# eBay/Sequence-Semantic-Embedding

Measured on AMD Instinct MI355X. Metric: encoded seqs/sec (+ query x target cosine-scores/sec, top-1 vs ref), higher is better.
Workload: dtype f32; 1 GPU; configs[1]: classification stand-in, dual-encoder LSTM H=S=256 E=50 T=32 V=32000; encode 16384 source seqs/GPU/step + cosine top-10 vs 571-target index; batch_per_gpu=16384, seq_len=32, targets=571, parallelism=dp1, weights=random-init (reference initialisers, seed 0)

## Files before the change

sequence-semantic-embedding_amd/csrc/score_topk.hip:

```cpp
#include <cstdlib>

#include "sse_kernels.h"
#include "score_exact.h"

#define SC_THREADS 512
#define SC_KC 16
#ifndef SC_PRIO_K
#define SC_PRIO_K 1
#define SC_PRIO_E 0
#endif

#ifdef SSE_SCORE_CLOCK
#include <cstdio>
__device__ long long g_score_clk[8 * 8];
#define SC_CLK_DECL long long ck_[8] = {0, 0, 0, 0, 0, 0, 0, 0}, ck_t = clock64();
#define SC_CLK(i)                   \
  {                                 \
    const long long n_ = clock64(); \
    ck_[i] += n_ - ck_t;            \
    ck_t = n_;                      \
  }
#else
#define SC_CLK_DECL
#define SC_CLK(i)
// ... 798 lines not shown
    const int64_t blk = i >> 6;
    const int kb = (int)(blk % KB);
    const int64_t tile = blk / KB;
    const int kg = kb * 2 + (l >> 5), r = l & 31;
    f32x4 lo4 = {0, 0, 0, 0}, hi4 = {0, 0, 0, 0};
    if (kg < KG) {
      lo4 = in[((size_t)tile * KG + kg) * 64 + r];
      hi4 = in[((size_t)tile * KG + kg) * 64 + 32 + r];
    }
    const float v[8] = {lo4[0], lo4[1], lo4[2], lo4[3], hi4[0], hi4[1], hi4[2], hi4[3]};
    sse_u32x4 h, lw;
    sse_split8(v, h, lw);
    out[(size_t)blk * 128 + l] = h;
    out[(size_t)blk * 128 + 64 + l] = lw;
  }
}

hipError_t launch_frag32_to_split_bf16(const float *idxp, int64_t NT, int KG, void *out, hipStream_t stream) {
  const int KB = (KG + 1) / 2;
  const int64_t total8 = NT * KB * 64;
  if (total8 == 0) return hipSuccess;
  const int64_t blocks = (total8 + 255) / 256;
  hipLaunchKernelGGL(frag32_to_split_bf16_kernel, dim3((int)(blocks < 16384 ? blocks : 16384)), dim3(256), 0, stream,
                     reinterpret_cast<const f32x4 *>(idxp), KG, KB, total8, reinterpret_cast<sse_u32x4 *>(out));
  return hipGetLastError();
}

__device__ __forceinline__ int si_key(float f) {
  const int i = __float_as_int(f);
  return i >= 0 ? i : (i ^ 0x7FFFFFFF);
}
__device__ __forceinline__ float si_val(int k) { return __int_as_float(k >= 0 ? k : (k ^ 0x7FFFFFFF)); }
template <int CTRL, int ROWMASK>
__device__ __forceinline__ float dpp_f(float x) {
  return __int_as_float(__builtin_amdgcn_update_dpp(__float_as_int(x), __float_as_int(x), CTRL, ROWMASK, 0xF, false));
}
__device__ __forceinline__ float wave_max_f(float x) {
  x = fmaxf(x, dpp_f<0x128, 0xF>(x));
  x = fmaxf(x, dpp_f<0x124, 0xF>(x));
  x = fmaxf(x, dpp_f<0x122, 0xF>(x));
  x = fmaxf(x, dpp_f<0x121, 0xF>(x));
  x = fmaxf(x, dpp_f<0x142, 0xA>(x));
  x = fmaxf(x, dpp_f<0x143, 0xC>(x));
  return __int_as_float(__builtin_amdgcn_readlane(__float_as_int(x), 63));
}
template <int JMAX>
#ifdef SSE_SCORE_CLOCK
#define SI_CLK_PARAMS , long long (&ck_)[8], long long &ck_t
#define SI_CLK_ARGS , ck_, ck_t
#else
#define SI_CLK_PARAMS
#define SI_CLK_ARGS
#endif
__device__ __forceinline__ void si_select4(const SmallIndexArgs &a, const float *sc, int NP, int NT, int qt, int q0, int lane SI_CLK_PARAMS) {
  constexpr int QW = 4;
  const int J = (NT * 32 + 63) / 64;
  float v[QW][JMAX];
#pragma unroll
  for (int j = 0; j < JMAX; ++j) {
    const int row = lane + 64 * j;
#pragma unroll
    for (int c = 0; c < QW; ++c) v[c][j] = (j < J && row < NT * 32) ? sc[(q0 + c) * NP + row] : NEG_INF;
  }
  int lok[QW], hik[QW];
  float lm[QW];
  bool done[QW];
#pragma unroll
  for (int c = 0; c < QW; ++c) {
    float m = NEG_INF;
#pragma unroll
    for (int j = 0; j < JMAX; ++j) m = fmaxf(m, v[c][j]);
    lm[c] = m;
    lok[c] = si_key(-wave_max_f(-m));
    hik[c] = si_key(wave_max_f(m)) + 1;
    done[c] = false;
  }
  SC_CLK(5)
  for (;;) {
    bool all_done = true;
#pragma unroll
    for (int c = 0; c < QW; ++c) {
      const unsigned width = (unsigned)hik[c] - (unsigned)lok[c];
      const int mid = lok[c] + (int)(width >> 1);
      const int cnt = __popcll(__ballot(lm[c] >= si_val(mid)));
      const bool open = !done[c] && width > 1u;
      const bool ge = cnt >= SC_KC;
      lok[c] = (open && ge) ? mid : lok[c];
      hik[c] = (open && !ge) ? mid : hik[c];
      done[c] = !open || (ge && cnt <= 24);
      all_done = all_done && done[c];
    }
    if (all_done) break;
  }
  SC_CLK(6)
#pragma unroll
  for (int c = 0; c < QW; ++c) {
    const int query = qt * 32 + q0 + c;
    if (query < a.Q) {
      const float T = si_val(lok[c]);
      float cs = NEG_INF;
      int cr = -1, base = 0;
#pragma unroll
      for (int j = 0; j < JMAX; ++j) {
        const bool take = (j < J) & (v[c][j] >= T) & (v[c][j] > NEG_INF);
        const unsigned long long mask = __ballot(take);
        const int n = __popcll(mask);
        const int slot = base + (int)__builtin_amdgcn_mbcnt_hi((unsigned)(mask >> 32), __builtin_amdgcn_mbcnt_lo((unsigned)mask, 0u));
        const int dst = (take && slot < 63) ? slot : 63;
        const int gs = __builtin_amdgcn_ds_permute(dst * 4, __float_as_int(v[c][j]));
        const int gr = __builtin_amdgcn_ds_permute(dst * 4, lane + 64 * j);
        const bool recv = (lane >= base) & (lane < base + n) & (lane < 63);
        cs = recv ? __int_as_float(gs) : cs;
        cr = recv ? gr : cr;
        base += n;
      }
      const int nw = base < 63 ? base : 63;
      int rank = 0;
      for (int l = 0; l < nw; ++l) {
        const float os = __int_as_float(__builtin_amdgcn_readlane(__float_as_int(cs), l));
        const int orow = __builtin_amdgcn_readlane(cr, l);
        rank += ((os > cs) | ((os == cs) & (orow < cr))) ? 1 : 0;
      }
      const bool mine = lane < nw;
      if (mine && rank < SC_KC) {
        a.part_scores[(size_t)query * SC_KC + rank] = cs;
        a.part_ids[(size_t)query * SC_KC + rank] = cr;
      }
      if (lane >= nw && lane < SC_KC) {
        a.part_scores[(size_t)query * SC_KC + lane] = NEG_INF;
        a.part_ids[(size_t)query * SC_KC + lane] = -1;
      }
      const unsigned long long m16 = __ballot(mine && rank == SC_KC - 1);
      const float last = m16 ? __int_as_float(__builtin_amdgcn_readlane(__float_as_int(cs), __ffsll((long long)m16) - 1)) : NEG_INF;
      if (lane == 0) a.part_bnd[query] = (base > 63) ? __builtin_inff() : last;
    }
  }
}

template <int KGC>
__global__ __launch_bounds__(256) void score_small_index_kernel(SmallIndexArgs a) {
  extern __shared__ __attribute__((aligned(16))) float si_sc[];
  const int tid = threadIdx.x, lane = tid & 63, w = __builtin_amdgcn_readfirstlane(tid >> 6);
  const int NT = a.NT, NP = NT * 32 + 1;
  const int qt = blockIdx.x;
  float *sc = si_sc;
  SC_CLK_DECL
  f32x4 b[KGC];
  {
    const int row = qt * 32 + (lane & 31), kb = (lane >> 5) * 4;
    const float *src = a.q_rows + (size_t)(row < a.Q ? row : 0) * a.S + kb;
    const bool vec = (a.S & 3) == 0 && (reinterpret_cast<uintptr_t>(a.q_rows) & 15) == 0 && KGC * 8 <= a.S;
#pragma unroll
    for (int kg = 0; kg < KGC; ++kg) {
      f32x4 v = {0, 0, 0, 0};
      if (vec) {
        v = *reinterpret_cast<const f32x4 *>(src + kg * 8);
      } else {
#pragma unroll
        for (int e = 0; e < 4; ++e)
          if (kg * 8 + kb + e < a.S) v[e] = src[kg * 8 + e];
      }
      if (row >= a.Q) v = f32x4{0, 0, 0, 0};
      b[kg] = v;
    }
  }
  SC_CLK(0)
  for (int t = w; t < NT; t += 4) {
    const f32x4 *ap = reinterpret_cast<const f32x4 *>(a.idxp) + (size_t)t * KGC * 64 + lane;
    f32x16 acc = {0, 0, 0, 0, 0, 0, 0, 0, 0, 0, 0, 0, 0, 0, 0, 0};
    f32x4 ar[4];
#pragma unroll
    for (int d = 0; d < 4; ++d) ar[d] = ap[(d < KGC ? d : 0) * 64];
#pragma unroll
    for (int kg = 0; kg < KGC; ++kg) {
      __builtin_amdgcn_sched_barrier(0);
#pragma unroll
      for (int e = 0; e < 4; ++e) acc = __builtin_amdgcn_mfma_f32_32x32x2f32(ar[kg & 3][e], b[kg][e], acc, 0, 0, 0);
      __builtin_amdgcn_sched_barrier(0);
      ar[kg & 3] = ap[(kg + 4 < KGC ? kg + 4 : kg) * 64];
    }
    const int rb = t * 32 + 4 * (lane >> 5);
    float *col = sc + (lane & 31) * NP;
#pragma unroll
    for (int r = 0; r < 16; ++r) {
      const int row = rb + (r & 3) + 8 * (r >> 2);
      col[row] = (row < a.N) ? acc[r] : NEG_INF;
    }
  }
  SC_CLK(1)
  __syncthreads();
  SC_CLK(2)
  if (NT * 32 <= 640) {
    si_select4<10>(a, sc, NP, NT, qt, w * 8, lane SI_CLK_ARGS);
    SC_CLK(3)
    si_select4<10>(a, sc, NP, NT, qt, w * 8 + 4, lane SI_CLK_ARGS);
    SC_CLK(4)
#ifdef SSE_SCORE_CLOCK
    if (blockIdx.x == gridDim.x / 2 && lane == 0)
      for (int i = 0; i < 8; ++i) g_score_clk[w * 8 + i] = ck_[i];
#endif
  } else {
    si_select4<16>(a, sc, NP, NT, qt, w * 8, lane SI_CLK_ARGS);
    si_select4<16>(a, sc, NP, NT, qt, w * 8 + 4, lane SI_CLK_ARGS);
  }
}
template <int KB>
__global__ __launch_bounds__(256) void score_small_index_x3_kernel(SmallIndexArgs a) {
  extern __shared__ __attribute__((aligned(16))) float si_sc[];
  const int tid = threadIdx.x, lane = tid & 63, w = __builtin_amdgcn_readfirstlane(tid >> 6);
  const int NT = a.NT, NP = NT * 32 + 1;
  const int qt = blockIdx.x;
  float *sc = si_sc;
  SC_CLK_DECL
  sse_u32x4 bh[KB], bl[KB];
  {
    const int row = qt * 32 + (lane & 31), kb0 = (lane >> 5) * 8;
    const float *src = a.q_rows + (size_t)(row < a.Q ? row : 0) * a.S + kb0;
    const bool vec = (a.S & 3) == 0 && (reinterpret_cast<uintptr_t>(a.q_rows) & 15) == 0 && KB * 16 <= a.S;
#pragma unroll
    for (int kb = 0; kb < KB; ++kb) {
      float v[8] = {0, 0, 0, 0, 0, 0, 0, 0};
      if (vec) {
        const f32x4 v0 = *reinterpret_cast<const f32x4 *>(src + kb * 16), v1 = *reinterpret_cast<const f32x4 *>(src + kb * 16 + 4);
#pragma unroll
        for (int e = 0; e < 4; ++e) {
          v[e] = v0[e];
          v[4 + e] = v1[e];
        }
      } else {
#pragma unroll
        for (int e = 0; e < 8; ++e)
          if (kb * 16 + kb0 + e < a.S) v[e] = src[kb * 16 + e];
      }
      if (row >= a.Q) {
#pragma unroll
        for (int e = 0; e < 8; ++e) v[e] = 0.0f;
      }
      sse_split8(v, bh[kb], bl[kb]);
    }
  }
  SC_CLK(0)
  {
    constexpr int D = KB < 4 ? KB : 4;
    static_assert(KB % D == 0, "the ring index must be static");
    const sse_u32x4 *img = reinterpret_cast<const sse_u32x4 *>(a.idx_x3) + lane;
    const sse_u32x4 *ap = img + (size_t)(w < NT ? w : 0) * KB * 128;
    sse_u32x4 ah[D], al[D];
#pragma unroll
    for (int d = 0; d < D; ++d) {
      ah[d] = ap[d * 128];
      al[d] = ap[d * 128 + 64];
    }
    for (int t = w; t < NT; t += 4) {
      const sse_u32x4 *apn = img + (size_t)(t + 4 < NT ? t + 4 : t) * KB * 128;
      f32x16 acc = {0, 0, 0, 0, 0, 0, 0, 0, 0, 0, 0, 0, 0, 0, 0, 0};
#pragma unroll
      for (int kb = 0; kb < KB; ++kb) {
        __builtin_amdgcn_sched_barrier(0);
        const bf16x8_t xh = __builtin_bit_cast(bf16x8_t, ah[kb % D]), xl = __builtin_bit_cast(bf16x8_t, al[kb % D]);
        const bf16x8_t yh = __builtin_bit_cast(bf16x8_t, bh[kb]), yl = __builtin_bit_cast(bf16x8_t, bl[kb]);
        acc = __builtin_amdgcn_mfma_f32_32x32x16_bf16(xh, yh, acc, 0, 0, 0);
        acc = __builtin_amdgcn_mfma_f32_32x32x16_bf16(xh, yl, acc, 0, 0, 0);
        acc = __builtin_amdgcn_mfma_f32_32x32x16_bf16(xl, yh, acc, 0, 0, 0);
        __builtin_amdgcn_sched_barrier(0);
        const sse_u32x4 *nx = (kb + D < KB) ? ap + (kb + D) * 128 : apn + (kb + D - KB) * 128;
        ah[kb % D] = nx[0];
        al[kb % D] = nx[64];
      }
      const int rb = t * 32 + 4 * (lane >> 5);
      float *col = sc + (lane & 31) * NP;
#pragma unroll
      for (int r = 0; r < 16; ++r) {
        const int row = rb + (r & 3) + 8 * (r >> 2);
        col[row] = (row < a.N) ? acc[r] : NEG_INF;
      }
      ap = apn;
    }
  }
  SC_CLK(1)
  __syncthreads();
  SC_CLK(2)
  if (NT * 32 <= 640) {
    si_select4<10>(a, sc, NP, NT, qt, w * 8, lane SI_CLK_ARGS);
    SC_CLK(3)
    si_select4<10>(a, sc, NP, NT, qt, w * 8 + 4, lane SI_CLK_ARGS);
    SC_CLK(4)
#ifdef SSE_SCORE_CLOCK
    if (blockIdx.x == gridDim.x / 2 && lane == 0)
      for (int i = 0; i < 8; ++i) g_score_clk[w * 8 + i] = ck_[i];
#endif
  } else {
    si_select4<16>(a, sc, NP, NT, qt, w * 8, lane SI_CLK_ARGS);
    si_select4<16>(a, sc, NP, NT, qt, w * 8 + 4, lane SI_CLK_ARGS);
  }
}
bool score_small_index_applies(int Q, int KG, int64_t NT) {
  return Q >= 1024 && (KG == 32 || KG == 8 || KG == 7) && NT * 32 <= 1024 && (size_t)32 * (NT * 32 + 1) * sizeof(float) <= (size_t)144 * 1024;
}
hipError_t launch_score_small_index(const SmallIndexArgs &a, hipStream_t stream) {
  if (!score_small_index_applies(a.Q, a.KG, a.NT)) return hipErrorInvalidValue;
  const size_t lds = (size_t)32 * (a.NT * 32 + 1) * sizeof(float);
  const dim3 grid((a.Q + 31) / 32), block(256);
  auto go = [&](auto kernel) -> hipError_t {
    hipError_t e = hipFuncSetAttribute(reinterpret_cast<const void *>(kernel), hipFuncAttributeMaxDynamicSharedMemorySize, (int)lds);
    if (e != hipSuccess) return e;
    hipLaunchKernelGGL(kernel, grid, block, lds, stream, a);
    return hipGetLastError();
  };
  if (a.idx_x3 && a.KG != 32) return go(score_small_index_x3_kernel<4>);
  if (a.KG == 8) return go(score_small_index_kernel<8>);
  if (a.KG == 7) return go(score_small_index_kernel<7>);
  const hipError_t e32 = a.idx_x3 ? go(score_small_index_x3_kernel<16>) : go(score_small_index_kernel<32>);
  if (e32 != hipSuccess) return e32;
#ifdef SSE_SCORE_CLOCK
  if (a.Q >= 8192) {
    static int n = 0;
    if (n++ % 8 == 3) {
      long long v[64];
      (void)hipStreamSynchronize(stream);
      (void)hipMemcpyFromSymbol(v, HIP_SYMBOL(g_score_clk), sizeof v);
      for (int w = 0; w < 4; w += 3)
        fprintf(stderr, "[small index clock Q=%d NT=%d] wave %d cycles: query fragments %lld | scores (MFMA + LDS stores) %lld | barrier %lld | selection: loads + bounds %lld | bisection %lld | winners + rank + stores %lld (both batches)\n",
                a.Q, a.NT, w, v[w * 8 + 0], v[w * 8 + 1], v[w * 8 + 2], v[w * 8 + 5], v[w * 8 + 6], v[w * 8 + 3] + v[w * 8 + 4]);
    }
  }
#endif
  return hipGetLastError();
}

hipError_t launch_score_topk(const ScoreArgs &a_in, hipStream_t stream) {
  ScoreArgs a = a_in;
#ifdef SSE_SCORE_MEASURE
  {
    static const int dbg = getenv("SSE_SCORE_DBG") ? atoi(getenv("SSE_SCORE_DBG")) : 0;
    a.dbg = dbg;
  }
#endif
  if (a.KC != SC_KC) return hipErrorInvalidValue;
  if (a.q_rows && ((a.NQ != 1 && !a.COLLECT) || a.S < 1)) return hipErrorInvalidValue;
  if (a.NSPLIT > 8 && (a.NSPLIT & 7)) return hipErrorInvalidValue;
  if (a.NSPLIT < 8 && (8 % a.NSPLIT)) return hipErrorInvalidValue;
  if (a.COLLECT) {
    if (!a.lane_max && (!a.col_thr || !a.col_slot || !a.col_cnt || !a.col_buf)) return hipErrorInvalidValue;
    if (a.BF) return a.NQ == 4 ? launch_score_variant<4, true, true>(a, stream) : hipErrorInvalidValue;
    if (a.NQ == 1) return launch_score_variant<1, false, true>(a, stream);
    if (a.NQ == 2) return launch_score_variant<2, false, true>(a, stream);
    if (a.NQ == 4) return launch_score_variant<4, false, true>(a, stream);
    return hipErrorInvalidValue;
  }
  if (!a.part_bnd) return hipErrorInvalidValue;
  if (a.BF) {
    if (a.NQ == 1) return launch_score_variant<1, true, false>(a, stream);
    if (a.NQ == 2) return launch_score_variant<2, true, false>(a, stream);
    if (a.NQ == 4) return launch_score_variant<4, true, false>(a, stream);
    return hipErrorInvalidValue;
  }
  if (a.NQ == 1) return launch_score_variant<1, false, false>(a, stream);
  if (a.NQ == 2) return launch_score_variant<2, false, false>(a, stream);
  if (a.NQ == 4) return launch_score_variant<4, false, false>(a, stream);
  return hipErrorInvalidValue;
}


template <int NB>
__device__ __forceinline__ int packed_value_of_lane(int lane) {
  int v = 0;
#pragma unroll
  for (int cnt = NB, bit = 5; cnt > 1; cnt >>= 1, --bit) v = v * 2 + ((lane >> bit) & 1);
  return v;
}
template <int NB>
__device__ __forceinline__ int packed_lane_of_value(int v) {
  int lane = 0;
#pragma unroll
  for (int cnt = NB, bit = 5; cnt > 1; cnt >>= 1, --bit) lane |= ((v / (cnt / 2)) & 1) << bit;
  return lane;
}
template <int NB>
__device__ __forceinline__ double wave_exact_dot_packed(const float *qrow, const float *idxp, const double *idx64, const int64_t (&n)[NB],
                                                        int S, int KG, int lane, const float *idx_rm = nullptr) {
  static_assert(NB == 2 || NB == 4 || NB == 8, "power of two");
  double acc[NB];
#pragma unroll
  for (int b = 0; b < NB; ++b) acc[b] = 0.0;
  if (idx64) {
    for (int d = lane; d < S; d += 64) {
      double rv[NB];
#pragma unroll
      for (int b = 0; b < NB; ++b) rv[b] = idx64[(size_t)n[b] * S + d];
#pragma unroll
      for (int b = 0; b < NB; ++b) acc[b] += (double)qrow[d] * rv[b];
    }
  } else {
    for (int j = lane; j < KG * 2; j += 64) {
      const int kg = j >> 1, half = j & 1;
      f32x4 v[NB];
#pragma unroll
      for (int b = 0; b < NB; ++b)
        v[b] = idx_rm ? *reinterpret_cast<const f32x4 *>(idx_rm + (size_t)n[b] * S + j * 4)
                      : *reinterpret_cast<const f32x4 *>(idxp + (size_t)(n[b] >> 5) * KG * 256 + kg * 256 + (half * 32 + (int)(n[b] & 31)) * 4);
      const int d0 = kg * 8 + half * 4;
#pragma unroll
      for (int e = 0; e < 4; ++e)
        if (d0 + e < S) {
#pragma unroll
          for (int b = 0; b < NB; ++b) acc[b] += (double)qrow[d0 + e] * (double)v[b][e];
        }
    }
  }
  int m = 32;
#pragma unroll
  for (int cnt = NB; cnt > 1; cnt >>= 1, m >>= 1) {
    const bool up = (lane & m) != 0;
#pragma unroll
    for (int i = 0; i < cnt / 2; ++i) {
      const double send = up ? acc[i] : acc[i + cnt / 2];
      const double keep = up ? acc[i + cnt / 2] : acc[i];
      acc[i] = keep + __shfl_xor(send, m);
    }
  }
#pragma unroll
  for (; m > 0; m >>= 1) acc[0] += __shfl_xor(acc[0], m);
  return acc[0];
}

#define RS_THREADS 256
#define RS_MAXWIN 256
#define RS_MAXNC 4096
__global__ __launch_bounds__(RS_THREADS) void rescore_kernel(RescoreArgs a) {
  __shared__ int s_cnt;
  __shared__ int s_wid[RS_MAXWIN];
  __shared__ double s_ex[RS_MAXWIN];
  __shared__ float s_m[RS_THREADS / 64];
  __shared__ double s_qn[RS_THREADS / 64];
  extern __shared__ __attribute__((aligned(16))) unsigned long long s_key[];
  const int q = blockIdx.x, tid = threadIdx.x, lane = tid & 63, w = tid >> 6;
  if (a.uncert_clear && q == 0 && tid == 0) *a.uncert_clear = 0;
  if (a.q_count && q >= *a.q_count) return;
  const int qo = a.qmap ? a.qmap[q] : q;
  const float *ps = a.part_scores + (size_t)q * a.NC;
  const int32_t *pi = a.part_ids + (size_t)q * a.NC;
  const float *qrow = a.q + (size_t)q * a.S;
  const int KG = (a.S + 7) / 8;

  constexpr int PER = RS_MAXNC / RS_THREADS;
  float rs[PER];
  int ri[PER];
#pragma unroll
  for (int j = 0; j < PER; ++j) {
    const int c = tid + j * RS_THREADS;
    ri[j] = (c < a.NC) ? pi[c] : -1;
    rs[j] = (c < a.NC) ? ps[c] : NEG_INF;
  }
  float mmax = NEG_INF;
  for (int c = tid; c < a.NC / SC_KC; c += RS_THREADS) mmax = fmaxf(mmax, a.part_bnd[(size_t)q * (a.NC / SC_KC) + c]);

  {
    double v = 0.0;
    for (int d = tid; d < a.S; d += RS_THREADS) v += (double)qrow[d] * qrow[d];
#pragma unroll
    for (int o = 32; o > 0; o >>= 1) v += __shfl_xor(v, o);
    if (lane == 0) s_qn[w] = v;
  }
#pragma unroll
  for (int o = 32; o > 0; o >>= 1) mmax = fmaxf(mmax, __shfl_xor(mmax, o));
  if (lane == 0) s_m[w] = mmax;
  if (tid == 0) s_cnt = 0;

#pragma unroll
  for (int j = 0; j < PER; ++j) {
    const int c = tid + j * RS_THREADS;
    if (c < a.NC) {
      unsigned u = __float_as_uint(rs[j]);
      u = (u & 0x80000000u) ? ~u : (u | 0x80000000u);
      s_key[c] = (ri[j] < 0) ? 0ull : (((unsigned long long)u << 32) | (unsigned long long)(0xFFFFFFFFu - (unsigned)ri[j]));
    }
// ... 82 lines not shown
#pragma unroll
    for (int c = 0; c < 4; ++c) n[c] = s_wid[min(i0 + c, nwin - 1)];
    const double tot = wave_exact_dot_packed<4>(qrow, a.idx32, a.idx64, n, a.S, KG, lane, a.idx_rm);
    const int c = packed_value_of_lane<4>(lane);
    if ((lane & 15) == 0 && i0 + c < nwin) s_ex[i0 + c] = tot;
  }
  __syncthreads();

  double theta = -__builtin_inf();
  for (int i = tid; i < nwin; i += RS_THREADS) {
    const double s = s_ex[i];
    const int64_t id = s_wid[i];
    int rank = 0;
    for (int j = 0; j < nwin; ++j) rank += before(s_ex[j], (int64_t)s_wid[j], s, id);
    if (rank < a.k) {
      a.out_scores[(size_t)qo * a.k + rank] = s;
      a.out_ids[(size_t)qo * a.k + rank] = a.id_base + id;
      if (a.host_flag) {
        a.host_scores[(size_t)qo * a.k + rank] = s;
        a.host_ids[(size_t)qo * a.k + rank] = a.id_base + id;
      }
    }
    if (rank == a.k - 1) theta = s;
  }
  if (a.host_flag) __threadfence_system();
  {
    double t = theta;
#pragma unroll
    for (int o = 32; o > 0; o >>= 1) t = fmax(t, __shfl_xor(t, o));
    __syncthreads();
    if (lane == 0) s_ex[w] = t;
    __syncthreads();
    if (tid == 0) {
      t = fmax(fmax(s_ex[0], s_ex[1]), fmax(s_ex[2], s_ex[3]));
      const bool ok = (nwin_all <= RS_MAXWIN) && (nwin >= a.k) && ((double)mmax + (double)eps_q < t);
      a.cert[qo] = ok ? 1 : 0;
      if (!ok && a.uncert) atomicAdd(a.uncert, 1);
      if (a.col_thr) a.col_thr[qo] = ok ? __builtin_inff() : __double2float_rd(t - (double)(a.eps32 * qnorm));
      if (a.col_slot) {
        a.col_slot[qo] = ok ? -1 : qo;
        a.col_cnt[qo] = 0;
      }
      if (a.host_flag) {
        a.host_cert[qo] = ok ? 1 : 0;
        if (qo == 0 && a.host_err) *a.host_err = a.err_in ? *a.err_in : 0;
        __hip_atomic_store(a.host_flag + qo, a.seq, __ATOMIC_RELEASE, __HIP_MEMORY_SCOPE_SYSTEM);
      }
    }
  }
}

#ifndef RS_NB
#define RS_NB 4
#endif
__device__ __forceinline__ double readlane_f64(double v, int l) {
  const long long b = __double_as_longlong(v);
  const int lo = __builtin_amdgcn_readlane((int)b, l), hi = __builtin_amdgcn_readlane((int)(b >> 32), l);
  return __longlong_as_double(((long long)hi << 32) | (unsigned int)lo);
}
__global__ __launch_bounds__(256) void rescore_small_kernel(RescoreArgs a) {
  const int lane = threadIdx.x & 63;
  const int q = blockIdx.x * 4 + (threadIdx.x >> 6);
  if (a.uncert_clear && blockIdx.x == 0 && threadIdx.x == 0) *a.uncert_clear = 0;
  if (q >= a.Q) return;
  if (a.q_count && q >= *a.q_count) return;
  const int qo = a.qmap ? a.qmap[q] : q;
  const float *qrow = a.q + (size_t)q * a.S;
  const int KG = (a.S + 7) / 8;
#ifdef SSE_SCORE_CLOCK
  long long rk_[6] = {0, 0, 0, 0, 0, 0}, rk_t = clock64();
#define RS_CLK(i) { const long long n_ = clock64(); rk_[i] += n_ - rk_t; rk_t = n_; }
#else
#define RS_CLK(i)
#endif
  const bool have = lane < a.NC;
  const int id = have ? a.part_ids[(size_t)q * a.NC + lane] : -1;
  const float sc = have ? a.part_scores[(size_t)q * a.NC + lane] : NEG_INF;
  const float bnd = (lane < a.NC / SC_KC) ? a.part_bnd[(size_t)q * (a.NC / SC_KC) + lane] : NEG_INF;
  double qn = 0.0;
  for (int d = lane; d < a.S; d += 64) qn += (double)qrow[d] * qrow[d];
#pragma unroll
  for (int o = 32; o > 0; o >>= 1) qn += __shfl_xor(qn, o);
  const float qnorm = (float)sqrt(qn);
  const float eps_q = a.eps * qnorm;
  RS_CLK(0)

  unsigned u = __float_as_uint(sc);
  u = (u & 0x80000000u) ? ~u : (u | 0x80000000u);
  const unsigned long long key = (id < 0) ? 0ull : (((unsigned long long)u << 32) | (unsigned long long)(0xFFFFFFFFu - (unsigned)id));
  const int key_lo = (int)(unsigned)key, key_hi = (int)(unsigned)(key >> 32);
  int rank = 0;
  for (int j = 0; j < a.NC; ++j) {
    const unsigned long long kj = ((unsigned long long)(unsigned)__builtin_amdgcn_readlane(key_hi, j) << 32) |
                                  (unsigned long long)(unsigned)__builtin_amdgcn_readlane(key_lo, j);
    rank += (kj > key) ? 1 : 0;
  }
  const unsigned long long kmask = __ballot(key != 0ull && rank == a.k - 1);
  const float kth = kmask ? __int_as_float(__builtin_amdgcn_readlane(__float_as_int(sc), __ffsll((long long)kmask) - 1)) : NEG_INF;
  const bool in_win = (id >= 0) && (sc >= kth - 2.0f * eps_q);
  float mmax = NEG_INF;
  for (int j = 0; j < a.NC / SC_KC; ++j) mmax = fmaxf(mmax, __int_as_float(__builtin_amdgcn_readlane(__float_as_int(bnd), j)));
  const unsigned long long wmask = __ballot(in_win);
  const int nwin = __popcll(wmask);
  const int mi = __popcll(wmask & ((1ull << lane) - 1ull));
  const int idm = __builtin_amdgcn_ds_permute((in_win ? mi : 63) * 4, id);
  RS_CLK(1)
  double exm = -__builtin_inf();
  for (int m0 = 0; m0 < nwin; m0 += RS_NB) {
    int64_t n[RS_NB];
#pragma unroll
    for (int c = 0; c < RS_NB; ++c) n[c] = __builtin_amdgcn_readlane(idm, (m0 + c < nwin) ? m0 + c : 0);
    const double tot = wave_exact_dot_packed<RS_NB>(qrow, a.idx32, a.idx64, n, a.S, KG, lane, a.idx_rm);
    const int want = lane - m0;
    const double got = __shfl(tot, packed_lane_of_value<RS_NB>(want & (RS_NB - 1)));
    if (want >= 0 && want < RS_NB && lane < nwin) exm = got;
  }
  RS_CLK(2)
  int r2 = 0;
  for (int j = 0; j < nwin; ++j)
    r2 += before(readlane_f64(exm, j), (int64_t)__builtin_amdgcn_readlane(idm, j), exm, (int64_t)idm) ? 1 : 0;
  const bool member = lane < nwin;
  if (member && r2 < a.k) {
    a.out_scores[(size_t)qo * a.k + r2] = exm;
    a.out_ids[(size_t)qo * a.k + r2] = a.id_base + idm;
    if (a.host_flag) {
      a.host_scores[(size_t)qo * a.k + r2] = exm;
      a.host_ids[(size_t)qo * a.k + r2] = a.id_base + idm;
    }
  }
  const unsigned long long tmask = __ballot(member && r2 == a.k - 1);
  const double theta = tmask ? readlane_f64(exm, __ffsll((long long)tmask) - 1) : -__builtin_inf();
  if (a.host_flag) __threadfence_system();
  RS_CLK(3)
#ifdef SSE_SCORE_CLOCK
  if (q == a.Q / 2 && lane == 0) {
    rk_[4] = nwin;
    for (int i = 0; i < 6; ++i) g_score_clk[i] = rk_[i];
  }
#endif
  if (lane == 0) {
    const bool ok = (nwin >= a.k) && ((double)mmax + (double)eps_q < theta);
    a.cert[qo] = ok ? 1 : 0;
    if (!ok && a.uncert) atomicAdd(a.uncert, 1);
    if (a.col_thr) a.col_thr[qo] = ok ? __builtin_inff() : __double2float_rd(theta - (double)(a.eps32 * qnorm));
    if (a.col_slot) {
      a.col_slot[qo] = ok ? -1 : qo;
      a.col_cnt[qo] = 0;
    }
    if (a.host_flag) {
      a.host_cert[qo] = ok ? 1 : 0;
      if (qo == 0 && a.host_err) *a.host_err = a.err_in ? *a.err_in : 0;
      __hip_atomic_store(a.host_flag + qo, a.seq, __ATOMIC_RELEASE, __HIP_MEMORY_SCOPE_SYSTEM);
    }
  }
}

hipError_t launch_rescore(const RescoreArgs &a, hipStream_t stream) {
  if (a.NC > RS_MAXNC) return hipErrorInvalidValue;
  if (a.NC <= 64) {
    hipLaunchKernelGGL(rescore_small_kernel, dim3((a.Q + 3) / 4), dim3(256), 0, stream, a);
// ... 366 lines not shown
```

sequence-semantic-embedding_amd/csrc/sse_api.hip:

```cpp
#include <cmath>
#include <cstdarg>
#include <cstdio>
#include <cstdlib>
#include <algorithm>
#include <chrono>
#include <cstring>
#include <dlfcn.h>
#include <link.h>
#include <mutex>
#include <string>
#include <vector>

#include "../../include/sse_hip.h"
#include "sse_kernels.h"
#include "train.h"

namespace {

thread_local std::string g_create_error;

struct Variable {
  std::string name;
  int rows = 0, cols = 0;
  int64_t count = 0;
// ... 1534 lines not shown
  a.N = h->idx_N;
  a.Q = Q;
  a.KG = bf ? KG16 : KG;
  a.NT = (int)NT;
  a.QT = QT;
  a.NSPLIT = nsplit;
  a.KC = 16;
  a.NQ = NQ;
  if (first) {
    if (small_idx) {
      SmallIndexArgs si{q, h->idxp, a.part_scores, a.part_ids, a.part_bnd, h->idx_N, Q, S, KG, (int)NT};
      if (small_x3) si.idx_x3 = h->idx_x3.p;
      HIPCHECK(h, launch_score_small_index(si, st));
    } else {
      HIPCHECK(h, launch_score_topk(a, st));
    }
  }
  RescoreArgs r;
  r.q = q;
  r.idx32 = h->idxp;
  r.idx64 = h->idx64;
  r.idx_rm = h->idx_rm_valid ? (const float *)h->idx_rm.p : nullptr;
  r.part_scores = a.part_scores;
  r.part_ids = a.part_ids;
  r.part_bnd = a.part_bnd;
  r.out_scores = out_s;
  r.out_ids = out_i;
  r.cert = (int32_t *)h->s_cert.p;
  r.id_base = h->idx_base;
  r.N = h->idx_N;
  r.Q = Q;
  r.S = S;
  r.NC = NC;
  r.k = k;
  const float eps32 = (float)(2.0 * (S + 2) * 5.97e-8 * h->idx_norm_max);
  r.eps = eps32;
  r.eps32 = eps32;
  r.col_thr = (float *)h->s_cthr.p;
  if (first) h->uncert_word ^= 1;
  int32_t *const uncert = (int32_t *)(counters + 4) + h->uncert_word;
  const int follow_grid = 2 * (h->cu_count > 0 ? h->cu_count : 256);
  r.uncert = uncert;
  r.uncert_clear = (int32_t *)(counters + 4) + (h->uncert_word ^ 1);
  const bool own_slots = Q <= POOL;
  if (own_slots) {
    r.col_slot = (int32_t *)h->s_cslot.p;
    r.col_cnt = (int32_t *)h->s_ccnt.p;
  }
  if (bf) r.eps += (float)(1.02 * (1.0 / 256.0 + 1.0 / 262144.0) * h->idx_norm_max);
  if (small_x3)
    r.eps = (float)(((1.0 + 1.0 / 64.0) / 32768.0 + 2.0 * (3 * S + 2) * 5.97e-8 * (1.0 + 1.0 / 32.0)) * h->idx_norm_max);
  if (first) {
    RescoreArgs rf = r;
    if (mirror) {
      rf.host_scores = mirror->scores;
      rf.host_ids = mirror->ids;
      rf.host_cert = mirror->cert;
      rf.host_err = mirror->err;
      rf.host_flag = mirror->flag;
      rf.err_in = h->err_flag;
      rf.seq = mirror->seq;
    }
    HIPCHECK(h, launch_rescore(rf, st));
  }
  if (!rest) return 0;
  const float *qp32 = (const float *)h->s_qp.p;
  if (bf && Q > 32) {
    if (reserve(h, h->s_qp32, (size_t)QB * NQ * KG * 256 * sizeof(float))) return 1;
    if (reserve(h, h->s_qmap, (size_t)(Q + 1) * sizeof(int32_t))) return 1;
    if (reserve(h, h->s_qc, (size_t)QT * 32 * S * sizeof(float))) return 1;
    HIPCHECK(h, launch_count_uncert(r.cert, Q, counters, st));
    int32_t *qmap = (int32_t *)h->s_qmap.p, *qcount = qmap + Q;
    HIPCHECK(h, launch_compact_uncert(q, r.cert, Q, S, qmap, qcount, (float *)h->s_qc.p, st));
    if (!rows_direct) HIPCHECK(h, launch_pack_rows((const float *)h->s_qc.p, Q, S, (float *)h->s_qp32.p, st));
    ScoreArgs a2 = a;
    a2.BF = 0;
    a2.idxp = h->idxp;
    a2.qp = (const float *)h->s_qp32.p;
    if (rows_direct) a2.q_rows = (const float *)h->s_qc.p;
    a2.KG = KG;
    a2.q_count = qcount;
    a2.NSPLIT = nsplit2;
    HIPCHECK(h, launch_score_topk(a2, st));
    RescoreArgs r2 = r;
    r2.q = (const float *)h->s_qc.p;
    r2.NC = nsplit2 * 16;
    r2.eps = eps32;
    r2.qmap = qmap;
    r2.q_count = qcount;
    r2.uncert = r2.uncert_clear = nullptr;
    HIPCHECK(h, launch_rescore(r2, st));
    qp32 = (const float *)h->s_qp32.p;
  }
  if (!own_slots) {
    HIPCHECK(h, hipMemsetAsync(h->s_ccnt.p, 0, (size_t)(POOL + 1) * sizeof(int32_t), st));
    HIPCHECK(h, launch_assign_slots(r.cert, Q, POOL, (int32_t *)h->s_cslot.p, (int32_t *)h->s_ccnt.p + POOL, st));
  }
  ScoreArgs c = a;
  c.BF = 0;
  c.idxp = h->idxp;
  c.qp = qp32;
  c.q_rows = q;
  c.S = S;
  c.KG = KG;
  c.COLLECT = 1;
  c.col_thr = (const float *)h->s_cthr.p;
// ... 2000 lines not shown
```

sequence-semantic-embedding_amd/csrc/sse_kernels.h:

```cpp
#pragma once
#include <hip/hip_runtime.h>
#include <stdint.h>

typedef float f32x4 __attribute__((ext_vector_type(4)));
typedef float f32x16 __attribute__((ext_vector_type(16)));

__host__ __device__ static inline int frag32_off(int r_in_tile, int k_in_group) {
  return ((((k_in_group >> 2) << 5) + r_in_tile) << 2) + (k_in_group & 3);
}

__device__ static inline int mfma_row(int reg, int lane) { return (reg & 3) + 8 * (reg >> 2) + 4 * (lane >> 5); }

static inline int round_up(int x, int m) { return (x + m - 1) / m * m; }

typedef unsigned int sse_u32x4 __attribute__((ext_vector_type(4)));
__host__ __device__ static inline unsigned short sse_bf16_rne(float f) {
  unsigned u;
  __builtin_memcpy(&u, &f, 4);
  u += 0x7FFFu + ((u >> 16) & 1u);
  return (unsigned short)(u >> 16);
}
__host__ __device__ static inline float sse_bf16_f32(unsigned short h) {
  const unsigned u = (unsigned)h << 16;
  float f;
// ... 205 lines not shown
  int32_t BF = 0;
  int32_t COLLECT = 0;
  const float *col_thr = nullptr;
  const int32_t *col_slot = nullptr;
  int32_t *col_cnt = nullptr;
  int32_t *col_buf = nullptr;
  int32_t col_cap = 0;
  float *lane_max = nullptr;
  int32_t dbg = 0;
  const float *q_rows = nullptr;
  int32_t S = 0;
  const int32_t *uncert = nullptr;
};
hipError_t launch_score_topk(const ScoreArgs &a, hipStream_t stream);
hipError_t launch_lane_max_threshold(const float *q, const float *lane_max, int Q, int S, int NV, float eps, float *col_thr,
                                     int32_t *col_slot, hipStream_t st);
#define SSE_MAX_INDEX_DIM 1024
int score_pick_nq(int Q, int S, int with_bf16);
size_t score_lds_bytes(int NQ, int KG, int BF, int COLLECT);
hipError_t launch_pack_rows_bf16(const float *rows, int64_t R, int C, void *out, hipStream_t stream);
hipError_t launch_count_uncert(const int32_t *cert, int Q, unsigned long long *count, hipStream_t st);
hipError_t launch_compact_uncert(const float *q, const int32_t *cert, int Q, int S, int32_t *qmap, int32_t *count, float *qc,
                                 hipStream_t st);
hipError_t launch_frag32_to_bf16(const float *idxp, int64_t NT, int KG, void *out, hipStream_t stream);
hipError_t launch_frag32_to_split_bf16(const float *idxp, int64_t NT, int KG, void *out, hipStream_t stream);

#define SSE_COLLECT_CAP 4096
#define SSE_MAX_SELECT_K 1024

struct RescoreArgs {
  const float *q;
  const float *idx32;
  const double *idx64;
  const float *part_scores;
  const int32_t *part_ids;
  const float *part_bnd;
  double *out_scores;
  int64_t *out_ids;
  int32_t *cert;
  int64_t id_base, N;
  int32_t Q, S, NC, k;
  float eps;
  const int32_t *qmap = nullptr, *q_count = nullptr;
  float *col_thr = nullptr;
  float eps32 = 0.0f;
  int32_t *col_slot = nullptr, *col_cnt = nullptr;
  double *host_scores = nullptr;
  int64_t *host_ids = nullptr;
  int32_t *host_cert = nullptr, *host_flag = nullptr, *host_err = nullptr;
  const int32_t *err_in = nullptr;
  int32_t seq = 0;
  const float *idx_rm = nullptr;
  int32_t *uncert = nullptr, *uncert_clear = nullptr;
};
hipError_t launch_rescore(const RescoreArgs &a, hipStream_t stream);

struct SmallIndexArgs {
  const float *q_rows;
  const float *idxp;
  float *part_scores;
  int32_t *part_ids;
  float *part_bnd;
  int64_t N;
  int32_t Q, S, KG, NT;
  const void *idx_x3 = nullptr;
};
bool score_small_index_applies(int Q, int KG, int64_t NT);
hipError_t launch_score_small_index(const SmallIndexArgs &a, hipStream_t stream);

struct RankArgs {
  const float *q;
  const int32_t *pair_q;
  const int64_t *pair_id;
  const double *pair_score_in;
  const float *idxp;
  const double *idx64;
  int64_t *out_before;
  double *out_score;
  double *thr64;
  float *lo, *hi;
  unsigned long long *sure;
  int32_t *band_cnt, *band_buf;
  int32_t band_cap;
  const int32_t *bad;
  unsigned long long *counters;
  int64_t id_base, N;
  int32_t S, KG, NT, P, NSPLIT, NQ;
  float eps32;
};
hipError_t launch_rank_validate(const int32_t *pair_q, const int64_t *pair_id, int64_t L, int Q, int need_row, int64_t id_base,
                                int64_t N, int32_t *bad, int32_t *err_flag, hipStream_t st);
hipError_t launch_score_rank(const RankArgs &a, hipStream_t st);

struct AboveArgs {
  const float *q;
  const int32_t *pair_q;
  const double *pair_thr;
  const float *idxp;
  const double *idx64;
  float *lo, *hi;
  unsigned long long *sure;
  int32_t *band_cnt, *band_buf;
  int32_t band_cap;
  const int32_t *bad;
  int32_t *err_flag;
  unsigned long long *counters;
// ... 150 lines not shown
```

Measured before the change: 7.614 million seqs/s.

## Restructure small-index top-k select, query fragment staging, and rescore prefetch

After: 7.620 million seqs/s (median of 3 runs). Within noise of the previous version (+0.1%).

```diff
diff --git a/sequence-semantic-embedding_amd/csrc/score_topk.hip b/sequence-semantic-embedding_amd/csrc/score_topk.hip
--- a/sequence-semantic-embedding_amd/csrc/score_topk.hip
+++ b/sequence-semantic-embedding_amd/csrc/score_topk.hip
@@ -874,7 +874,7 @@
 #define SI_CLK_PARAMS
 #define SI_CLK_ARGS
 #endif
-__device__ __forceinline__ void si_select4(const SmallIndexArgs &a, const float *sc, int NP, int NT, int qt, int q0, int lane SI_CLK_PARAMS) {
+__device__ __forceinline__ void si_select4(const SmallIndexArgs &a, float *sc, int NP, int NT, int qt, int q0, int lane SI_CLK_PARAMS) {
   constexpr int QW = 4;
   const int J = (NT * 32 + 63) / 64;
   float v[QW][JMAX];
@@ -915,46 +915,70 @@
     if (all_done) break;
   }
   SC_CLK(6)
+  float *const strip = NT >= 4 ? sc + q0 * NP : sc + 32 * NP + (q0 >> 3) * (QW * 128);
+  const int sstr = NT >= 4 ? NP : 128;
+  int base[QW];
+  float T[QW];
+#pragma unroll
+  for (int c = 0; c < QW; ++c) {
+    base[c] = 0;
+    T[c] = si_val(lok[c]);
+  }
+#pragma unroll
+  for (int j = 0; j < JMAX; ++j) {
+#pragma unroll
+    for (int c = 0; c < QW; ++c) {
+      const bool take = (j < J) & (v[c][j] >= T[c]) & (v[c][j] > NEG_INF);
+      const unsigned long long mask = __ballot(take);
+      const int slot = base[c] + (int)__builtin_amdgcn_mbcnt_hi((unsigned)(mask >> 32), __builtin_amdgcn_mbcnt_lo((unsigned)mask, 0u));
+      if (take && slot < 63) {
+        strip[c * sstr + slot] = v[c][j];
+        strip[c * sstr + 64 + slot] = __int_as_float(lane + 64 * j);
+      }
+      base[c] += __popcll(mask);
+    }
+  }
+  __builtin_amdgcn_fence(__ATOMIC_RELEASE, "wavefront");
+  __builtin_amdgcn_wave_barrier();
+  __builtin_amdgcn_fence(__ATOMIC_ACQUIRE, "wavefront");
+  int nw[QW], rank[QW], cr[QW], nmax = 0;
+  float cs[QW];
+  long long key[QW];
+#pragma unroll
+  for (int c = 0; c < QW; ++c) {
+    nw[c] = base[c] < 63 ? base[c] : 63;
+    nmax = nw[c] > nmax ? nw[c] : nmax;
+    const bool mine = lane < nw[c];
+    const float rs = strip[c * sstr + lane], rr = strip[c * sstr + 64 + lane];
+    cs[c] = mine ? rs : NEG_INF;
+    cr[c] = mine ? __float_as_int(rr) : -1;
+    key[c] = mine ? (long long)(((unsigned long long)(unsigned)si_key(cs[c] + 0.0f) << 32) | (unsigned)~cr[c]) : (long long)(1ull << 63);
+    rank[c] = 0;
+  }
+  for (int l = 0; l < nmax; ++l) {
+#pragma unroll
+    for (int c = 0; c < QW; ++c) {
+      const long long kl = (long long)(((unsigned long long)(unsigned)__builtin_amdgcn_readlane((int)(key[c] >> 32), l) << 32) |
+                                       (unsigned)__builtin_amdgcn_readlane((int)key[c], l));
+      rank[c] += (kl > key[c]) ? 1 : 0;
+    }
+  }
 #pragma unroll
   for (int c = 0; c < QW; ++c) {
     const int query = qt * 32 + q0 + c;
+    const bool mine = lane < nw[c];
+    const unsigned long long m16 = __ballot(mine && rank[c] == SC_KC - 1);
+    const float last = m16 ? __int_as_float(__builtin_amdgcn_readlane(__float_as_int(cs[c]), __ffsll((long long)m16) - 1)) : NEG_INF;
     if (query < a.Q) {
-      const float T = si_val(lok[c]);
-      float cs = NEG_INF;
-      int cr = -1, base = 0;
-#pragma unroll
-      for (int j = 0; j < JMAX; ++j) {
-        const bool take = (j < J) & (v[c][j] >= T) & (v[c][j] > NEG_INF);
-        const unsigned long long mask = __ballot(take);
-        const int n = __popcll(mask);
-        const int slot = base + (int)__builtin_amdgcn_mbcnt_hi((unsigned)(mask >> 32), __builtin_amdgcn_mbcnt_lo((unsigned)mask, 0u));
-        const int dst = (take && slot < 63) ? slot : 63;
-        const int gs = __builtin_amdgcn_ds_permute(dst * 4, __float_as_int(v[c][j]));
-        const int gr = __builtin_amdgcn_ds_permute(dst * 4, lane + 64 * j);
-        const bool recv = (lane >= base) & (lane < base + n) & (lane < 63);
-        cs = recv ? __int_as_float(gs) : cs;
-        cr = recv ? gr : cr;
-        base += n;
-      }
-      const int nw = base < 63 ? base : 63;
-      int rank = 0;
-      for (int l = 0; l < nw; ++l) {
-        const float os = __int_as_float(__builtin_amdgcn_readlane(__float_as_int(cs), l));
-        const int orow = __builtin_amdgcn_readlane(cr, l);
-        rank += ((os > cs) | ((os == cs) & (orow < cr))) ? 1 : 0;
-      }
-      const bool mine = lane < nw;
-      if (mine && rank < SC_KC) {
-        a.part_scores[(size_t)query * SC_KC + rank] = cs;
-        a.part_ids[(size_t)query * SC_KC + rank] = cr;
-      }
-      if (lane >= nw && lane < SC_KC) {
+      if (mine && rank[c] < SC_KC) {
+        a.part_scores[(size_t)query * SC_KC + rank[c]] = cs[c];
+        a.part_ids[(size_t)query * SC_KC + rank[c]] = cr[c];
+      }
+      if (lane >= nw[c] && lane < SC_KC) {
         a.part_scores[(size_t)query * SC_KC + lane] = NEG_INF;
         a.part_ids[(size_t)query * SC_KC + lane] = -1;
       }
-      const unsigned long long m16 = __ballot(mine && rank == SC_KC - 1);
-      const float last = m16 ? __int_as_float(__builtin_amdgcn_readlane(__float_as_int(cs), __ffsll((long long)m16) - 1)) : NEG_INF;
-      if (lane == 0) a.part_bnd[query] = (base > 63) ? __builtin_inff() : last;
+      if (lane == 0) a.part_bnd[query] = (base[c] > 63) ? __builtin_inff() : last;
     }
   }
 }
@@ -1036,14 +1060,16 @@
   SC_CLK_DECL
   sse_u32x4 bh[KB], bl[KB];
   {
-    const int row = qt * 32 + (lane & 31), kb0 = (lane >> 5) * 8;
-    const float *src = a.q_rows + (size_t)(row < a.Q ? row : 0) * a.S + kb0;
+    sse_u32x4 *frag = reinterpret_cast<sse_u32x4 *>(si_sc);
+    const int qi = w * 8 + (lane & 7), row = qt * 32 + qi;
+    const float *src = a.q_rows + (size_t)(row < a.Q ? row : 0) * a.S;
     const bool vec = (a.S & 3) == 0 && (reinterpret_cast<uintptr_t>(a.q_rows) & 15) == 0 && KB * 16 <= a.S;
 #pragma unroll
-    for (int kb = 0; kb < KB; ++kb) {
+    for (int i = 0; i < KB / 4; ++i) {
+      const int oc = (lane >> 3) + 8 * i;
       float v[8] = {0, 0, 0, 0, 0, 0, 0, 0};
       if (vec) {
-        const f32x4 v0 = *reinterpret_cast<const f32x4 *>(src + kb * 16), v1 = *reinterpret_cast<const f32x4 *>(src + kb * 16 + 4);
+        const f32x4 v0 = *reinterpret_cast<const f32x4 *>(src + oc * 8), v1 = *reinterpret_cast<const f32x4 *>(src + oc * 8 + 4);
 #pragma unroll
         for (int e = 0; e < 4; ++e) {
           v[e] = v0[e];
@@ -1052,14 +1078,24 @@
       } else {
 #pragma unroll
         for (int e = 0; e < 8; ++e)
-          if (kb * 16 + kb0 + e < a.S) v[e] = src[kb * 16 + e];
+          if (oc * 8 + e < a.S) v[e] = src[oc * 8 + e];
       }
       if (row >= a.Q) {
 #pragma unroll
         for (int e = 0; e < 8; ++e) v[e] = 0.0f;
       }
-      sse_split8(v, bh[kb], bl[kb]);
-    }
+      sse_u32x4 hi, lo;
+      sse_split8(v, hi, lo);
+      frag[(oc >> 1) * 128 + (oc & 1) * 32 + qi] = hi;
+      frag[(oc >> 1) * 128 + 64 + (oc & 1) * 32 + qi] = lo;
+    }
+    __syncthreads();
+#pragma unroll
+    for (int kb = 0; kb < KB; ++kb) {
+      bh[kb] = frag[kb * 128 + lane];
+      bl[kb] = frag[kb * 128 + 64 + lane];
+    }
+    __syncthreads();
   }
   SC_CLK(0)
   {
@@ -1121,7 +1157,9 @@
 }
 hipError_t launch_score_small_index(const SmallIndexArgs &a, hipStream_t stream) {
   if (!score_small_index_applies(a.Q, a.KG, a.NT)) return hipErrorInvalidValue;
-  const size_t lds = (size_t)32 * (a.NT * 32 + 1) * sizeof(float);
+  size_t lds = (size_t)32 * (a.NT * 32 + 1) * sizeof(float) + (a.NT < 4 ? (size_t)4 * 4 * 128 * sizeof(float) : 0);
+  const size_t frag = a.idx_x3 ? (size_t)(a.KG == 32 ? 16 : 4) * 2048 : 0;
+  if (lds < frag) lds = frag;
   const dim3 grid((a.Q + 31) / 32), block(256);
   auto go = [&](auto kernel) -> hipError_t {
     hipError_t e = hipFuncSetAttribute(reinterpret_cast<const void *>(kernel), hipFuncAttributeMaxDynamicSharedMemorySize, (int)lds);
@@ -1199,6 +1237,23 @@
   return lane;
 }
 template <int NB>
+__device__ __forceinline__ double packed_reduce(double (&acc)[NB], int lane) {
+  int m = 32;
+#pragma unroll
+  for (int cnt = NB; cnt > 1; cnt >>= 1, m >>= 1) {
+    const bool up = (lane & m) != 0;
+#pragma unroll
+    for (int i = 0; i < cnt / 2; ++i) {
+      const double send = up ? acc[i] : acc[i + cnt / 2];
+      const double keep = up ? acc[i + cnt / 2] : acc[i];
+      acc[i] = keep + __shfl_xor(send, m);
+    }
+  }
+#pragma unroll
+  for (; m > 0; m >>= 1) acc[0] += __shfl_xor(acc[0], m);
+  return acc[0];
+}
+template <int NB>
 __device__ __forceinline__ double wave_exact_dot_packed(const float *qrow, const float *idxp, const double *idx64, const int64_t (&n)[NB],
                                                         int S, int KG, int lane, const float *idx_rm = nullptr) {
   static_assert(NB == 2 || NB == 4 || NB == 8, "power of two");
@@ -1230,20 +1285,7 @@
         }
     }
   }
-  int m = 32;
-#pragma unroll
-  for (int cnt = NB; cnt > 1; cnt >>= 1, m >>= 1) {
-    const bool up = (lane & m) != 0;
-#pragma unroll
-    for (int i = 0; i < cnt / 2; ++i) {
-      const double send = up ? acc[i] : acc[i + cnt / 2];
-      const double keep = up ? acc[i + cnt / 2] : acc[i];
-      acc[i] = keep + __shfl_xor(send, m);
-    }
-  }
-#pragma unroll
-  for (; m > 0; m >>= 1) acc[0] += __shfl_xor(acc[0], m);
-  return acc[0];
+  return packed_reduce<NB>(acc, lane);
 }
 
 #define RS_THREADS 256
@@ -1432,6 +1474,9 @@
 
 #ifndef RS_NB
 #define RS_NB 4
+#endif
+#ifndef RS_PRE
+#define RS_PRE 4
 #endif
 __device__ __forceinline__ double readlane_f64(double v, int l) {
   const long long b = __double_as_longlong(v);
@@ -1457,6 +1502,14 @@
   const int id = have ? a.part_ids[(size_t)q * a.NC + lane] : -1;
   const float sc = have ? a.part_scores[(size_t)q * a.NC + lane] : NEG_INF;
   const float bnd = (lane < a.NC / SC_KC) ? a.part_bnd[(size_t)q * (a.NC / SC_KC) + lane] : NEG_INF;
+  const bool pre = !a.idx64 && KG * 2 <= 64;
+  const int pd0 = (lane >> 1) * 8 + (lane & 1) * 4;
+  float qv[4] = {0.0f, 0.0f, 0.0f, 0.0f};
+  if (pre && lane < KG * 2) {
+#pragma unroll
+    for (int e = 0; e < 4; ++e)
+      if (pd0 + e < a.S) qv[e] = qrow[pd0 + e];
+  }
   double qn = 0.0;
   for (int d = lane; d < a.S; d += 64) qn += (double)qrow[d] * qrow[d];
 #pragma unroll
@@ -1469,11 +1522,14 @@
   u = (u & 0x80000000u) ? ~u : (u | 0x80000000u);
   const unsigned long long key = (id < 0) ? 0ull : (((unsigned long long)u << 32) | (unsigned long long)(0xFFFFFFFFu - (unsigned)id));
   const int key_lo = (int)(unsigned)key, key_hi = (int)(unsigned)(key >> 32);
-  int rank = 0;
-  for (int j = 0; j < a.NC; ++j) {
-    const unsigned long long kj = ((unsigned long long)(unsigned)__builtin_amdgcn_readlane(key_hi, j) << 32) |
-                                  (unsigned long long)(unsigned)__builtin_amdgcn_readlane(key_lo, j);
-    rank += (kj > key) ? 1 : 0;
+  int rank = lane;
+  if (!a.sorted) {
+    rank = 0;
+    for (int j = 0; j < a.NC; ++j) {
+      const unsigned long long kj = ((unsigned long long)(unsigned)__builtin_amdgcn_readlane(key_hi, j) << 32) |
+                                    (unsigned long long)(unsigned)__builtin_amdgcn_readlane(key_lo, j);
+      rank += (kj > key) ? 1 : 0;
+    }
   }
   const unsigned long long kmask = __ballot(key != 0ull && rank == a.k - 1);
   const float kth = kmask ? __int_as_float(__builtin_amdgcn_readlane(__float_as_int(sc), __ffsll((long long)kmask) - 1)) : NEG_INF;
@@ -1486,6 +1542,46 @@
   const int idm = __builtin_amdgcn_ds_permute((in_win ? mi : 63) * 4, id);
   RS_CLK(1)
   double exm = -__builtin_inf();
+#if RS_PRE > 0
+  if (pre && nwin <= RS_PRE * RS_NB) {
+    f32x4 rv[RS_PRE * RS_NB];
+#pragma unroll
+    for (int bi = 0; bi < RS_PRE; ++bi) {
+      if (bi * RS_NB < nwin) {
+#pragma unroll
+        for (int c = 0; c < RS_NB; ++c) {
+          const int m = bi * RS_NB + c;
+          const int64_t n = __builtin_amdgcn_readlane(idm, (m < nwin) ? m : 0);
+          f32x4 x = {0, 0, 0, 0};
+          if (lane < KG * 2)
+            x = a.idx_rm ? *reinterpret_cast<const f32x4 *>(a.idx_rm + (size_t)n * a.S + lane * 4)
+                         : *reinterpret_cast<const f32x4 *>(a.idx32 + (size_t)(n >> 5) * KG * 256 + (lane >> 1) * 256 + ((lane & 1) * 32 + (int)(n & 31)) * 4);
+          rv[m] = x;
+        }
+      }
+    }
+#pragma unroll
+    for (int bi = 0; bi < RS_PRE; ++bi) {
+      if (bi * RS_NB < nwin) {
+        double acc[RS_NB];
+#pragma unroll
+        for (int c = 0; c < RS_NB; ++c) acc[c] = 0.0;
+        if (lane < KG * 2) {
+#pragma unroll
+          for (int e = 0; e < 4; ++e)
+            if (pd0 + e < a.S) {
+#pragma unroll
+              for (int c = 0; c < RS_NB; ++c) acc[c] += (double)qv[e] * (double)rv[bi * RS_NB + c][e];
+            }
+        }
+        const double tot = packed_reduce<RS_NB>(acc, lane);
+        const int want = lane - bi * RS_NB;
+        const double got = __shfl(tot, packed_lane_of_value<RS_NB>(want & (RS_NB - 1)));
+        if (want >= 0 && want < RS_NB && lane < nwin) exm = got;
+      }
+    }
+  } else
+#endif
   for (int m0 = 0; m0 < nwin; m0 += RS_NB) {
     int64_t n[RS_NB];
 #pragma unroll
diff --git a/sequence-semantic-embedding_amd/csrc/sse_api.hip b/sequence-semantic-embedding_amd/csrc/sse_api.hip
--- a/sequence-semantic-embedding_amd/csrc/sse_api.hip
+++ b/sequence-semantic-embedding_amd/csrc/sse_api.hip
@@ -1610,6 +1610,7 @@
     r.eps = (float)(((1.0 + 1.0 / 64.0) / 32768.0 + 2.0 * (3 * S + 2) * 5.97e-8 * (1.0 + 1.0 / 32.0)) * h->idx_norm_max);
   if (first) {
     RescoreArgs rf = r;
+    rf.sorted = (small_idx && NC == 16) ? 1 : 0;
     if (mirror) {
       rf.host_scores = mirror->scores;
       rf.host_ids = mirror->ids;
diff --git a/sequence-semantic-embedding_amd/csrc/sse_kernels.h b/sequence-semantic-embedding_amd/csrc/sse_kernels.h
--- a/sequence-semantic-embedding_amd/csrc/sse_kernels.h
+++ b/sequence-semantic-embedding_amd/csrc/sse_kernels.h
@@ -281,6 +281,7 @@
   int32_t seq = 0;
   const float *idx_rm = nullptr;
   int32_t *uncert = nullptr, *uncert_clear = nullptr;
+  int32_t sorted = 0;
 };
 hipError_t launch_rescore(const RescoreArgs &a, hipStream_t stream);
 
```
